# xyy7/Learning-based-RGB-D-Image-Compression

Measured on AMD Instinct MI355X. Metric: RGB-D Mpixels/s encode+decode, higher is better.
Workload: dtype f32; 1 GPU; c3_4x480x640; codec=ELIC_united ch4 q=2_2 (N=192,M=320), images_per_gpu=4, steps_per_call=4, images_per_call=16, calls=5, weights=synthetic seed 0 (stress recipe), streams=per image, y_bytes_last_batch=15943588, engine_instances=5, conv_tiles=throughput, warmup_steps_run=40, launch=HIP graph per call shape, pairs_in_flight=80

## Files before the change

### learning-based-rgb-d-image-compression_amd/csrc/common.h

```cpp
#pragma once
#include <hip/hip_runtime.h>
#include <stdint.h>
#include <stdio.h>

#define RGBD_OK 0
#define RGBD_EINVAL (-22)
#define RGBD_ENOMEM (-12)
#define RGBD_EHIP (-5)
#define RGBD_ENOSPC (-28)
#define RGBD_ESTATE (-1)

#define HIP_TRY(expr)                                                                          \
    do {                                                                                       \
        hipError_t _e = (expr);                                                                \
        if (_e != hipSuccess) {                                                                \
            fprintf(stderr, "[rgbd_amd] %s:%d %s -> %s\n", __FILE__, __LINE__, #expr,          \
                    hipGetErrorString(_e));                                                    \
            return RGBD_EHIP;                                                                  \
        }                                                                                      \
    } while (0)

struct Act {
    float* p = nullptr;
    int n = 0, h = 0, w = 0, c = 0, cs = 0;
// ... 101 lines not shown
    const long K = (long)cin_pad * taps_per_phase;
    int s;
    if (nphase == 1 && out_px_per_image <= 512) {
        if (taps_per_phase == 1) s = K >= 1500 ? 8 : (K >= 700 ? 4 : (K >= 350 ? 2 : 1));
        else s = K >= 5000 ? 8 : (K >= 1000 ? 4 : (K >= 500 ? 2 : 1));
    } else {
        s = (int)((K + 800) / 1600);
        if (s > 8) s = 8;
    }
    if (s > cin_pad / 16) s = cin_pad / 16;
    if (s < 1) s = 1;
    return s;
}

int launch_conv(const ConvArgs& a, hipStream_t s);
int conv_fused_plan(int cout_pad, int cout2_pad, int ntaps, int N, int GH, int GW, int loaded);
int launch_conv_fused(const ConvArgs& a, hipStream_t s);
int conv_log_enable(int on);
int conv_tile_override(const char* csv);
long conv_log_read(char* buf, long cap);
long conv_tile_list(int blocked, char* buf, long cap);

int launch_sigmoid_gate_ref(const float* t, int tcs, const float* mul, int mcs, const float* res2, int r2cs, float* y, int ycs,
                            int N, int HW, int C, int per_image, int threads, hipStream_t s);

int launch_nchw_to_nhwc16(const float* src, int N, int C, int H, int W, float* dst, int cs, hipStream_t s, int perm = 0);
int launch_nhwc_to_nchw_clamp(const float* src, int N, int C, int H, int W, int cs, float* dst, int clamp01,
                              hipStream_t s, int perm = 0);
int launch_maxpool7s3(const float* x, int N, int H, int W, int cs, float* y, int OH, int OW, hipStream_t s,
                      const float* x1 = nullptr, float* y1 = nullptr);
// ... 15 lines not shown
int launch_copy_channels(const float* src, int scs, float* dst, int dcs, int npix, int C, hipStream_t s);
struct SmallConvArgs {
    const float* x;
    const float* w;
    const float* bias;
    const float* res1;
    const float* mul;
    const float* res2;
    float* y;
    float* y2;
    int N, H, W, xcs, C, cin_pad, O, OH, OW, ycs, r1cs, mcs, r2cs, y2cs, K, stride, pad, act, nb;
    int ckbd;
    int kb[17];
};
int launch_small_conv_ref(const SmallConvArgs& a, hipStream_t s);
int launch_gather_taps(const float* x, int B, int h, int w, int cs, int j0, int jw, int ntap, const int* dy, const int* dx,
                       float* col, hipStream_t s);
int launch_gather_wslabs(const float* wp, int cout_pad, int ntaps_total, int cin_pad, int ntap, const int* slab, float* wout,
                         hipStream_t s);
int launch_scatter_phase(const float* src, int B, int h, int jw, int scs, int j0, int py, int px, float* dst, int OW, int dcs,
                         int C, hipStream_t s);
int launch_fill_zero(float* p, size_t n, hipStream_t s);
int launch_im2col5s2(const float* x, int N, int H, int W, int cs, int C, float* y, int OH, int OW, int KP, hipStream_t s);
int launch_layernorm(const float* x, size_t ntok, int C, int xcs, const float* w, const float* b, float* y, int ycs,
                     hipStream_t s, const float* x1 = nullptr, const float* w1 = nullptr, const float* b1 = nullptr,
                     float* y1 = nullptr);
int launch_window_attention(const float* qkv, int B, int H, int W, int C, int qcs, int heads, int shift, const float* rpb,
                            float* out, int ocs, hipStream_t s, const float* qkv1 = nullptr, const float* rpb1 = nullptr,
                            float* out1 = nullptr);
int launch_guided_window_attention(const float* q, int qcs, const float* kv, int kvcs, int B, int H, int W, int C, int heads,
                                   int shift, const float* rpb, float* out, int ocs, hipStream_t s);
int launch_patch_merge_gather(const float* x, int B, int H, int W, int C, int xcs, float* y, int ycs, hipStream_t s);
int launch_pixel_shuffle2(const float* x, int B, int H, int W, int Co, int xcs, float* y, int ycs, hipStream_t s);

struct GdnArgs {
    const float* x;
// ... 100 lines not shown
```

### learning-based-rgb-d-image-compression_amd/csrc/conv_mfma.hip

```cpp
#include <array>
#include <map>
#include <string>

#include "conv_mfma_body.h"
#include "conv_tiles.h"

bool conv_blk_tile_ok(int wm, int mt, int nt, int max_tiles);
int launch_conv_blk(const ConvArgs& a, const Choice& c, hipStream_t s);
int launch_conv_fused_blk(const ConvArgs& a, int cls, hipStream_t s);

namespace {

Choice choose(const ConvArgs& a, int max_tiles = 16)
{
    static const int cand[][3] = {{2, 3, 8}, {2, 2, 8}, {2, 5, 4}, {2, 4, 4}, {2, 3, 4}, {2, 2, 4}, {2, 1, 4}, {2, 5, 2}, {2, 4, 2},
                                  {2, 3, 2}, {2, 2, 2}, {2, 1, 2}, {2, 5, 1}, {2, 4, 1}, {2, 3, 1}, {2, 2, 1},
                                  {2, 1, 1}, {1, 3, 2}, {1, 2, 2}, {1, 1, 2}, {1, 3, 1}, {1, 2, 1}, {1, 1, 1}};
    int max_taps = 1;
    for (int p = 0; p < a.nphase; ++p) max_taps = a.taps.n[p] > max_taps ? a.taps.n[p] : max_taps;
    const double K = (double)max_taps * a.cin_pad / a.splitk;
    const int ck = a.ckbd ? 1 : 0;
    const int GWe = ck ? (a.GW + 1) / 2 : a.GW;
    Choice best{2, 4, 4, 16, 4, false};
    double best_cost = -1.0;
// ... 240 lines not shown
            p += used;
            ++n;
            if (*p == ',') ++p;
            else break;
        }
        while (*p && *p != '\n') ++p;
        if (*p == '\n') ++p;
        if (n != 14) return RGBD_EINVAL;
        char key[160];
        snprintf(key, sizeof(key), "%d,%d,%d,%d,%d,%d,%d,%d,%d", v[0], v[1], v[2], v[3], v[4], v[5], v[6], v[7], v[8]);
        g_ovr[key] = {v[9], v[10], v[11], v[12], v[13]};
    }
    return RGBD_OK;
}

int launch_conv(const ConvArgs& a_in, hipStream_t s)
{
    ConvArgs a = a_in;
    if (a.cout_store <= 0 || a.cout_store > a.cout_pad) a.cout_store = a.cout_pad;
    if (a.cout_store % 4) return RGBD_EINVAL;
    if (a.splitk < 1) a.splitk = 1;
    if (a.splitk > a.cin_pad / 16) a.splitk = a.cin_pad / 16;
    if (a.splitk > 1 && !a.partial) return RGBD_EINVAL;
    if (!conv_groups_ok(a)) return RGBD_EINVAL;
    {
        const size_t lim = (size_t)1 << 32;
        const size_t opx = (size_t)a.OH * a.OW * 4;
        const int ocs = std::max(std::max(a.ycs, a.cout_pad), std::max(a.r1cs, std::max(a.mcs, a.r2cs)));
        if ((size_t)a.H * a.W * a.xcs * 4 >= lim || opx * ocs >= lim ||
            (size_t)a.cout_pad * a.ntaps_total * a.cin_pad * 4 >= lim)
            return RGBD_EINVAL;
    }
    if (a.act == ACT_GELU && !a.partial) return RGBD_EINVAL;
    if (a.y2 && (a.partial || a.subpix || a.y2cs % 4)) return RGBD_EINVAL;
    if (a.subpix && (a.cout_pad != 16 || a.nphase != 1 || a.IS != 1 || a.OS != 2 || a.splitk > 1 || a.res1 || a.mul || a.res2 ||
                     a.ckbd || a.ycs < 4))
        return RGBD_EINVAL;
    if (a.ckbd && (a.ckbd > 2 || a.ckbd < 0 || a.nphase != 1 || a.IS != 1 || a.OS != 1)) return RGBD_EINVAL;
    const int rc = launch_conv_main(a, s);
    if (rc || !a.partial) return rc;
    const size_t total4 = (size_t)a.N * a.OH * a.OW * (a.cout_pad / 4);
    size_t g = ((a.groups == 2 ? 2 : 1) * total4 + 255) / 256;
    if (g > 2048) g = 2048;
    hipLaunchKernelGGL(splitk_reduce_kernel, dim3((unsigned)g), dim3(256), 0, s, a, total4);
    HIP_TRY(hipGetLastError());
    return RGBD_OK;
}

static int launch_conv_main(const ConvArgs& a, hipStream_t s)
{
    if (a.cin_pad % 16 || a.cout_pad % 16 || a.xcs % 4 || a.ycs % 4) return RGBD_EINVAL;
    if (a.nphase != 1 && a.nphase != 4) return RGBD_EINVAL;
    if (a.N <= 0 || a.GH <= 0 || a.GW <= 0) return RGBD_EINVAL;
    Choice c = choose(a);
    const TunedTile* t = tuned_lookup(a);
    if (t && a.blocked) {
        const int tiles = t->mt * t->nt;
        const bool ring = t->kc == 16 && (t->dma == 4 || t->dma == 5), dma = t->kc == 16 && t->dma != 0;
        if (!conv_blk_tile_ok(t->wm, t->mt, t->nt, 16) || (tiles > 12 && !ring) || (tiles > 10 && !dma)) t = nullptr;
    }
    if (t) {
// ... 103 lines not shown
```

### learning-based-rgb-d-image-compression_amd/csrc/engine.h

```cpp
#pragma once
#include <algorithm>
#include <array>
#include <cmath>
#include <cstdlib>
#include <cstring>
#include <functional>
#include <map>
#include <memory>
#include <mutex>
#include <shared_mutex>
#include <string>
#include <vector>

#include <atomic>
#include <chrono>
#include <condition_variable>
#include <dirent.h>
#include <execinfo.h>
#include <signal.h>
#include <sys/syscall.h>
#include <thread>
#include <unistd.h>

#include "../../include/rgbd_amd.h"
// ... 221 lines not shown
    int act = ACT_NONE;
    const Act* res1 = nullptr;
    const Act* mul = nullptr;
    const Act* res2 = nullptr;
    int ckbd = 0;
    const Act* dup = nullptr;
};


struct ArenaScratch {
    Arena& a;
    size_t mark() const { return a.top; }
    float* take(size_t bytes) { return (float*)a.take(bytes); }
    void release(size_t m) { a.top = m; }
};
template <class Scratch>
inline int deconv_s2_ref_run(const PackedConv& pcv, const int* rec, size_t nrec, const float* x, int B, int h, int w, int act,
                             float* out, int ocs, int tile_mode, bool launch, hipStream_t s, Scratch& scratch)
{
    const PackedConv* pc = &pcv;
    std::vector<const int*> desc(4 * (size_t)w, nullptr);
    {
        size_t pos = 0;
        for (size_t i = 0; i < desc.size(); ++i) {
            if (pos >= nrec || rec[pos] < 0 || (size_t)rec[pos] > (nrec - pos - 1) / 3) return RGBD_EINVAL;
            desc[i] = rec + pos;
            pos += 1 + 3 * (size_t)rec[pos];
        }
        if (pos != nrec) return RGBD_EINVAL;
    }
    auto same = [](const int* a, const int* b) { return a[0] == b[0] && memcmp(a, b, sizeof(int) * (1 + 3 * (size_t)a[0])) == 0; };
    for (int ph = 0; ph < 4; ++ph) {
        const int py = ph >> 1, px = ph & 1;
        for (int j0 = 0; j0 < w;) {
            const int* d = desc[(size_t)ph * w + j0];
            int j1 = j0 + 1;
            while (j1 < w && same(d, desc[(size_t)ph * w + j1])) ++j1;
            const int jw = j1 - j0, nt = d[0];
            if (nt < 1 || nt > 16) return RGBD_EINVAL;
            int dy[16], dx[16], slab[16], chain[16], nch = 0;
            for (int t = 0; t < nt; ++t) {
                const int ky = d[1 + 3 * t], kx = d[2 + 3 * t], fresh = d[3 + 3 * t];
                if (ky < 0 || ky > 4 || kx < 0 || kx > 4 || ((py + ky) & 1) || ((px + kx) & 1) || (fresh != 0 && fresh != 1)) return RGBD_EINVAL;
                dy[t] = (py + 2 - ky) / 2;
                dx[t] = (px + 2 - kx) / 2;
                slab[t] = ky * 5 + kx;
                if (fresh || t == 0) chain[nch++] = 0;
                chain[nch - 1] += pc->cin_pad;
            }
            const size_t mark = scratch.mark();
            const size_t npx = (size_t)B * h * jw;
            const int Kp = nt * pc->cin_pad;
            float* col = scratch.take(npx * Kp * sizeof(float));
            float* wsel = scratch.take((size_t)pc->cout_pad * Kp * sizeof(float));
            float* tmp = scratch.take(npx * pc->cout_pad * sizeof(float));
            float* part = nch > 1 ? scratch.take((size_t)nch * npx * pc->cout_pad * sizeof(float)) : nullptr;
            if (launch) {
                if (!col || !wsel || !tmp || (nch > 1 && !part)) return RGBD_ENOMEM;
                int r = launch_gather_taps(x, B, h, w, pc->cin_pad, j0, jw, nt, dy, dx, col, s);
                if (!r) r = launch_gather_wslabs(pc->w, pc->cout_pad, 25, pc->cin_pad, nt, slab, wsel, s);
                if (!r) {
                    PackedConv gemm;
                    gemm.w = wsel;
                    gemm.bias = pc->bias;
                    gemm.cin_pad = Kp;
                    gemm.cout_pad = pc->cout_pad;
                    gemm.k = 1;
                    ConvArgs a{};
                    conv_args_geometry(&a, gemm, col, 1, B * h, jw, Kp, tmp, pc->cout_pad, B * h, jw, 1, 0);
                    a.cout_store = pc->cout_pad;
                    a.act = act;
                    a.loaded = tile_mode;
                    a.exact_math = 1;
                    a.splitk = 1;
                    if (nch > 1) {
                        a.partial = part;
                        r = conv_set_split_ranges(&a, chain, nch);
                    }
                    if (!r) r = launch_conv(a, s);
                }
                if (!r) r = launch_scatter_phase(tmp, B, h, jw, pc->cout_pad, j0, py, px, out, 2 * w, ocs, pc->cout_pad, s);
                if (r) return r;
            }
            scratch.release(mark);
            j0 = j1;
        }
    }
    return RGBD_OK;
}

inline int small_conv_set_kblocks(SmallConvArgs* a, const int* lens, int n, int Kt)
{
    a->nb = 1;
    a->kb[0] = 0;
    a->kb[1] = Kt;
    if (!lens) return RGBD_OK;
    if (n < 1 || n > 16) return RGBD_EINVAL;
    int pos = 0;
    a->nb = n;
    for (int b = 0; b < n; ++b) {
        if (lens[b] <= 0 || lens[b] > Kt - pos) return RGBD_EINVAL;
        pos += lens[b];
        a->kb[b + 1] = pos;
// ... 20 lines not shown
        bool forward_names_z;
    };
    Modes modes() const
    {
        if (single()) return {1, {"", ""}, {"", ""}, {in_ch, in_ch}, variant == 4 ? 1 : 0, true};
        return {2, {"_r", "_d"}, {"rgb_", "depth_"}, {3, 1}, 1, false};
    }
    std::vector<int> slice_ch;
    std::map<std::string, HostTensor> raw;
    std::map<std::string, PackedConv> convs;
    std::map<std::string, float*> dense;
    TableSet tables[4];
    float* scale_table = nullptr;
    std::shared_ptr<DevGen> gen_w;
    std::shared_ptr<DevGen> gen_scale;
    bool finalized = false;

    Arena arena;
    hipStream_t s = nullptr;
    int rc = 0;
    std::map<std::string, Act> named;

    std::vector<std::vector<uint8_t>> streams[2][2];
    int32_t* dbg_sym = nullptr;
    int32_t* dbg_idx = nullptr;
    int64_t dbg_per_mod = 0;
    bool debug_floats = false;
    float* dbg_x = nullptr;
    float* dbg_s = nullptr;

// ... 1153 lines not shown
        const char* mods[2] = {"rgb", "depth"};
        const Act* in[2] = {&yr, &yd};
        Act* out[2] = {zr, zd};
        const std::string p[2] = {std::string("h_a.") + mods[0] + "_reduction.", std::string("h_a.") + mods[1] + "_reduction."};
        const Epi relu2[2] = {relu, relu}, none[2];
        const Act x0[2] = {*in[0], *in[1]};
        Act t0[2], t1[2], t2[2];
        const std::string n0[2] = {p[0] + "0", p[1] + "0"}, n2[2] = {p[0] + "2", p[1] + "2"}, n4[2] = {p[0] + "4", p[1] + "4"};
        conv2(2, n0, x0, 1, 1, relu2, nullptr, t0);
        conv2(2, n2, t0, 2, 2, relu2, nullptr, t1);
        conv2(2, n4, t1, 2, 2, none, nullptr, t2);
        *out[0] = t2[0];
        *out[1] = t2[1];
    }

    bool deconv_s2_ref(const std::string& name, const Act& x, int act, Act* out)
    {
        if (!refnum) return false;
        const PackedConv* pc = conv_of(name + ".weight");
        if (!pc || !pc->transposed || pc->k != 5 || pc->subpix || x.cs != pc->cin_pad) return false;
        const std::vector<int>* rec = ref_blocks(3, pc->cin, pc->cout, x.h, x.w);
        if (!rec) return false;
        *out = alloc(x.n, 2 * x.h, 2 * x.w, pc->cout);
        ArenaScratch scratch{arena};
        const int r = deconv_s2_ref_run(*pc, rec->data(), rec->size(), x.p, x.n, x.h, x.w, act, out->p, out->cs, tile_mode,
                                        !dry() && !rc, s, scratch);
        if (r) fail(r);
        return true;
    }

    void hs_block2(int nm, const std::string p[2], const Act own[2], const Act other[2], bool last, Act out[2])
    {
        Act f[2];
        std::string n[2];
        for (int m = 0; m < nm; ++m) {
            f[m] = alloc(own[m].n, own[m].h, own[m].w, own[m].c + other[m].c);
            se_cat_to(p[m] + ".se", own[m], other[m], f[m]);
            if (rc) return;
            n[m] = p[m] + ".deconv";
        }
        Epi e[2];
        e[0].act = e[1].act = last ? ACT_NONE : ACT_LEAKY;
        const PackedConv* pc0 = conv_of(n[0] + ".weight");
        if (nm == 2 && !last && refnum && pc0 && ref_blocks(3, pc0->cin, pc0->cout, f[0].h, f[0].w)) {
            bool ok = true;
            for (int m = 0; m < 2; ++m) ok = deconv_s2_ref(n[m], f[m], ACT_LEAKY, &out[m]) && ok;
            if (!ok) fail(RGBD_ESTATE);
            return;
        }
        conv2(nm, n, f, last ? 1 : 2, last ? 1 : 2, e, nullptr, out);
    }

    void h_s(const Act& zr, const Act& zd, Act* hr, Act* hd)
    {
        Act cur[2] = {zr, zd};
        for (int st = 1; st <= 3; ++st) {
            const std::string p[2] = {"h_s.r_h_s" + std::to_string(st), "h_s.d_h_s" + std::to_string(st)};
            const Act other[2] = {cur[1], cur[0]};
            Act o[2];
            hs_block2(2, p, cur, other, st == 3, o);
            cur[0] = o[0];
            cur[1] = o[1];
// ... 917 lines not shown
```

### learning-based-rgb-d-image-compression_amd/csrc/engine_abi.hip

```cpp
#include "engine.h"

extern "C" {

int rgbd_abi_version(void) { return RGBD_AMD_ABI_VERSION; }

static std::atomic<int> g_live_engines{0};
static std::mutex g_policy_mu;
static bool g_policy_done[64] = {false};

static int ensure_wait_policy()
{
    static const bool spin = getenv("RGBD_SPIN_WAIT") != nullptr;
    if (spin) return RGBD_OK;
    int dev = 0;
    HIP_TRY(hipGetDevice(&dev));
    std::lock_guard<std::mutex> g(g_policy_mu);
    if (dev < 0 || dev >= 64 || g_policy_done[dev]) return RGBD_OK;
    if (g_live_engines.load() == 0) {
        std::unique_lock<std::shared_mutex> cap_lk(g_capture_mu);
        HIP_TRY(hipDeviceSynchronize());
        HIP_TRY(hipSetDeviceFlags(hipDeviceScheduleBlockingSync));
    }
    g_policy_done[dev] = true;
    return RGBD_OK;
// ... 908 lines not shown
{
    if (!src || !out || !src->finalized) return RGBD_EINVAL;
    rgbd_elic* m = new rgbd_elic();
    m->N = src->N;
    m->M = src->M;
    m->slice_ch = src->slice_ch;
    m->variant = src->variant;
    m->in_ch = src->in_ch;
    m->out_ch = src->out_ch;
    m->refnum = src->refnum;
    m->ref_threads = src->ref_threads;
    m->ref_tab = src->ref_tab;
    m->convs = src->convs;
    m->dense = src->dense;
    m->gen_w = src->gen_w;
    for (int i = 0; i < 4; ++i) m->tables[i] = src->tables[i];
    m->scale_table = src->scale_table;
    m->scale_tab = src->scale_tab;
    m->gen_scale = src->gen_scale;
    m->finalized = true;
    m->is_clone = true;
    *out = m;
    ++g_live_engines;
    return RGBD_OK;
}

void rgbd_elic_destroy(rgbd_elic* m)
{
    const bool dbg = g_dbg_destroy;
    if (dbg) fprintf(stderr, "[destroy %p] wait lock\n", (void*)m);
// ... 66 lines not shown
    g->p.push_back(d);
    HIP_TRY(hipMemcpy(d, table, 64 * sizeof(float), hipMemcpyHostToDevice));
    m->scale_table = d;
    memcpy(m->scale_tab.v, table, sizeof(m->scale_tab.v));
    m->gen_scale = g;
    m->graphs_invalidate();
    return RGBD_OK;
}

static bool ends_with(const std::string& s, const char* suf)
{
    const size_t n = strlen(suf);
    return s.size() >= n && s.compare(s.size() - n, n, suf) == 0;
}

int rgbd_elic_set_ref_blocks(rgbd_elic* m, int32_t kind, int32_t cin, int32_t cout, int32_t h, int32_t w, int32_t batch,
                             const int32_t* blocks, int32_t nblocks)
{
    if (m && kind == 4 && blocks && nblocks == 1 && blocks[0] >= 1 && blocks[0] <= 4096) {
        m->ref_threads = blocks[0];
        m->graphs_invalidate();
        return RGBD_OK;
    }
    if (!m || !blocks || nblocks <= 0 || nblocks > (kind >= 2 ? 65536 : 64) || kind < 0 || kind > 3) return RGBD_EINVAL;
    int sum = 0;
    for (int i = 0; i < nblocks; ++i) {
        if (kind == 3 ? blocks[i] < 0 : (kind == 2 ? (blocks[i] < 0 || blocks[i] > 2) : blocks[i] <= 0)) return RGBD_EINVAL;
        sum += blocks[i];
    }
    if (kind == 0 && sum != cin) return RGBD_EINVAL;
    if (kind == 1 && nblocks > 16) return RGBD_EINVAL;
    if (kind == 2 && nblocks != cout) return RGBD_EINVAL;
    m->ref_tab->blocks[{kind, cin, cout, h, w, batch}] = std::vector<int>(blocks, blocks + nblocks);
    m->graphs_invalidate();
    return RGBD_OK;
}

int rgbd_elic_get_refnum(const rgbd_elic* m) { return m ? (m->refnum ? 1 : 0) : RGBD_EINVAL; }
int rgbd_elic_ref_table_misses(const rgbd_elic* m) { return m ? m->ref_tab->misses : RGBD_EINVAL; }

int rgbd_elic_finalize(rgbd_elic* m)
{
    std::unique_lock<std::shared_mutex> cap_lk(g_capture_mu);
    if (!m) return RGBD_EINVAL;
    if (m->is_clone && m->raw.empty()) return RGBD_ESTATE;
    auto gen = std::make_shared<DevGen>();
    std::map<std::string, PackedConv> convs;
    std::map<std::string, float*> dense;
    auto dev_copy = [&](const float* src, size_t n, float** out) -> int {
// ... 138 lines not shown
                const size_t no = (size_t)fi[i + 1], ni = (size_t)fi[i];
                if (mi->second.v.size() != C * no * ni || bi->second.v.size() != C * no || (i < 4 && fa->second.v.size() != C * no))
                    return RGBD_EINVAL;
                mat[i] = mi->second.v.data();
                bias[i] = bi->second.v.data();
                if (i < 4) fac[i] = fa->second.v.data();
            }
            if (ok) {
                eb_pack_cumulative(mat, bias, fac, C, prm.data());
                float* dp = nullptr;
                if (const int r = dev_copy(prm.data(), prm.size(), &dp)) return r;
                dense[pre + "cumulative"] = dp;
            }
        }
    }
    m->convs.swap(convs);
    m->dense.swap(dense);
    m->gen_w = gen;
    m->graphs_invalidate();
    m->finalized = true;
    return RGBD_OK;
}

static int check_ready(const rgbd_elic* m)
{
    if (m && m->variant == 6) return RGBD_EINVAL;
    if (!m || !m->finalized || !m->scale_table) return RGBD_ESTATE;
    for (int i = 0; i < 4; ++i)
        if (!m->tables[i].ready && !(m->single() && (i & 1))) return RGBD_ESTATE;
    return RGBD_OK;
}

int rgbd_elic_compress(rgbd_elic* m, const float* rgb_dev, const float* depth_dev, int32_t B, int32_t H, int32_t W,
// ... 246 lines not shown
```

### learning-based-rgb-d-image-compression_amd/csrc/pointwise.hip

```cpp
#include "common.h"
#include "exact_math.h"

typedef float f32x4 __attribute__((ext_vector_type(4)));

static inline unsigned grid_for(size_t work, int block = 256, unsigned cap = 256 * 8)
{
    size_t g = (work + block - 1) / block;
    if (g > cap) g = cap;
    if (g < 1) g = 1;
    return (unsigned)g;
}

__global__ void nchw_to_nhwc16_kernel(const float* __restrict__ src, int N, int C, int H, int W, float* __restrict__ dst,
                                      int cs, int perm)
{
    const size_t npix = (size_t)N * H * W;
    const int c4n = cs / 4;
    for (size_t i = blockIdx.x * (size_t)blockDim.x + threadIdx.x; i < npix * c4n; i += (size_t)gridDim.x * blockDim.x) {
        const size_t pix = i / c4n;
        const int c4 = (int)(i - pix * c4n);
        const size_t hw = pix % ((size_t)H * W);
        const size_t n = pix / ((size_t)H * W);
        f32x4 v;
#pragma unroll
// ... 517 lines not shown

int launch_se_fc_ref(const float* mean, int N, int C, int hidden, const float* w0, const float* w1, const int* cls0,
                     const int* cls1, float* hid, float* scale, hipStream_t s, int mstride, int form)
{
    const int r = launch_se_linear_ref(w0, mean, N, C, hidden, mstride > 0 ? mstride : C, 1, cls0, ACT_RELU, hid, hidden, 0, form, s);
    if (r) return r;
    return launch_se_linear_ref(w1, hid, N, hidden, C, hidden, 0, cls1, ACT_SIGMOID, scale, C, 1, form, s);
}

struct TapList {
    int n;
    int8_t dy[16], dx[16];
    uint8_t slab[16];
};

__global__ void gather_taps_kernel(const float* __restrict__ x, int B, int h, int w, int cs, int j0, int jw, TapList tl,
                                   float* __restrict__ col)
{
    const int c4n = cs / 4;
    const size_t total = (size_t)B * h * jw * tl.n * c4n;
    for (size_t i = blockIdx.x * (size_t)blockDim.x + threadIdx.x; i < total; i += (size_t)gridDim.x * blockDim.x) {
        const int c4 = (int)(i % c4n);
        size_t r = i / c4n;
        const int t = (int)(r % tl.n);
        r /= tl.n;
        const int tx = (int)(r % jw);
        r /= jw;
        const int ty = (int)(r % h);
        const size_t n = r / h;
        const int iy = ty + tl.dy[t], ix = j0 + tx + tl.dx[t];
        f32x4 v = (f32x4){0.f, 0.f, 0.f, 0.f};
        if (iy >= 0 && iy < h && ix >= 0 && ix < w) v = *reinterpret_cast<const f32x4*>(x + ((n * h + iy) * (size_t)w + ix) * cs + c4 * 4);
        *reinterpret_cast<f32x4*>(col + (((n * h + ty) * (size_t)jw + tx) * tl.n + t) * cs + c4 * 4) = v;
    }
}

__global__ void gather_wslabs_kernel(const float* __restrict__ wp, int cout_pad, int ntaps_total, int cin_pad, TapList tl,
                                     float* __restrict__ wout)
{
    const int c4n = cin_pad / 4;
    const size_t total = (size_t)cout_pad * tl.n * c4n;
    for (size_t i = blockIdx.x * (size_t)blockDim.x + threadIdx.x; i < total; i += (size_t)gridDim.x * blockDim.x) {
        const int c4 = (int)(i % c4n);
        size_t r = i / c4n;
        const int t = (int)(r % tl.n);
        const size_t co = r / tl.n;
        *reinterpret_cast<f32x4*>(wout + (co * tl.n + t) * cin_pad + c4 * 4) =
            *reinterpret_cast<const f32x4*>(wp + (co * ntaps_total + tl.slab[t]) * cin_pad + c4 * 4);
    }
}

__global__ void scatter_phase_kernel(const float* __restrict__ src, int B, int h, int jw, int scs, int j0, int py, int px,
                                     float* __restrict__ dst, int OW, int dcs, int c4n)
{
    const size_t total = (size_t)B * h * jw * c4n;
    for (size_t i = blockIdx.x * (size_t)blockDim.x + threadIdx.x; i < total; i += (size_t)gridDim.x * blockDim.x) {
        const int c4 = (int)(i % c4n);
        size_t r = i / c4n;
        const int tx = (int)(r % jw);
        r /= jw;
        const int ty = (int)(r % h);
        const size_t n = r / h;
        *reinterpret_cast<f32x4*>(dst + ((n * 2 * h + 2 * ty + py) * (size_t)OW + 2 * (j0 + tx) + px) * dcs + c4 * 4) =
            *reinterpret_cast<const f32x4*>(src + ((n * h + ty) * (size_t)jw + tx) * scs + c4 * 4);
    }
}

int launch_gather_taps(const float* x, int B, int h, int w, int cs, int j0, int jw, int ntap, const int* dy, const int* dx,
                       float* col, hipStream_t s)
{
    if (ntap < 1 || ntap > 16 || cs % 4) return RGBD_EINVAL;
    TapList tl{};
    tl.n = ntap;
    for (int t = 0; t < ntap; ++t) tl.dy[t] = (int8_t)dy[t], tl.dx[t] = (int8_t)dx[t];
    const size_t work = (size_t)B * h * jw * ntap * (cs / 4);
    hipLaunchKernelGGL(gather_taps_kernel, dim3(grid_for(work)), dim3(256), 0, s, x, B, h, w, cs, j0, jw, tl, col);
    HIP_TRY(hipGetLastError());
    return RGBD_OK;
}

int launch_gather_wslabs(const float* wp, int cout_pad, int ntaps_total, int cin_pad, int ntap, const int* slab, float* wout,
                         hipStream_t s)
{
    if (ntap < 1 || ntap > 16 || cin_pad % 4) return RGBD_EINVAL;
    TapList tl{};
    tl.n = ntap;
    for (int t = 0; t < ntap; ++t) tl.slab[t] = (uint8_t)slab[t];
    const size_t work = (size_t)cout_pad * ntap * (cin_pad / 4);
    hipLaunchKernelGGL(gather_wslabs_kernel, dim3(grid_for(work)), dim3(256), 0, s, wp, cout_pad, ntaps_total, cin_pad, tl, wout);
    HIP_TRY(hipGetLastError());
    return RGBD_OK;
}

int launch_scatter_phase(const float* src, int B, int h, int jw, int scs, int j0, int py, int px, float* dst, int OW, int dcs,
                         int C, hipStream_t s)
{
    if (C % 4 || scs % 4 || dcs % 4) return RGBD_EINVAL;
    const size_t work = (size_t)B * h * jw * (C / 4);
    hipLaunchKernelGGL(scatter_phase_kernel, dim3(grid_for(work)), dim3(256), 0, s, src, B, h, jw, scs, j0, py, px, dst, OW, dcs, C / 4);
    HIP_TRY(hipGetLastError());
    return RGBD_OK;
}


__global__ void sigmoid_gate_ref_kernel(const float* __restrict__ t, int tcs, const float* __restrict__ mul, int mcs,
                                        const float* __restrict__ res2, int r2cs, float* __restrict__ y, int ycs, int N, int HW,
                                        int C, int per_image, int threads)
{
    const int C16 = (C + 15) & ~15;
    const size_t total = (size_t)N * HW * C16;
    const long numel = (long)(per_image ? 1 : N) * C * HW;
    for (size_t i = blockIdx.x * (size_t)blockDim.x + threadIdx.x; i < total; i += (size_t)gridDim.x * blockDim.x) {
        const int sc = (int)(i % C16);
        const size_t pix = i / C16;
// ... 26 lines not shown
```

Measured before the change: 18.89 Mpx/s.

## Batch stride-2 deconv classes into grouped gather, paired GEMMs, fused finish kernel

Restructures the reference stride-2 transposed-conv path so all phase/column classes are gathered by one grouped kernel per 16 classes instead of one launch each. The two modalities run as a paired GEMM group that writes split partials. A single finish kernel sums the partials, adds bias, applies the activation and scatters into the output, replacing the per-class split-k reduce and scatter launches. Weight slabs can come from a prebuilt cache set at finalize, which removes the per-call gather_wslabs. This cuts kernel launch count and per-class scratch reuse, at the cost of more simultaneous scratch memory for all classes.

New measurement: 18.80 Mpx/s (median of 2 runs). No clear change (-0.5%).

```diff
diff --git a/learning-based-rgb-d-image-compression_amd/csrc/common.h b/learning-based-rgb-d-image-compression_amd/csrc/common.h
--- a/learning-based-rgb-d-image-compression_amd/csrc/common.h
+++ b/learning-based-rgb-d-image-compression_amd/csrc/common.h
@@ -139,6 +139,7 @@
 }
 
 int launch_conv(const ConvArgs& a, hipStream_t s);
+int launch_conv_partials(const ConvArgs& a, hipStream_t s);
 int conv_fused_plan(int cout_pad, int cout2_pad, int ntaps, int N, int GH, int GW, int loaded);
 int launch_conv_fused(const ConvArgs& a, hipStream_t s);
 int conv_log_enable(int on);
@@ -184,12 +185,24 @@
     int kb[17];
 };
 int launch_small_conv_ref(const SmallConvArgs& a, hipStream_t s);
-int launch_gather_taps(const float* x, int B, int h, int w, int cs, int j0, int jw, int ntap, const int* dy, const int* dx,
-                       float* col, hipStream_t s);
+struct DeconvClass {
+    int j0, jw, nt;
+    int py, px;
+    int planes;
+    unsigned long long col_off, part_off;
+    int8_t dy[16], dx[16];
+};
+struct DeconvClassTab {
+    static constexpr int kMax = 16;
+    int n;
+    DeconvClass c[kMax];
+};
+int launch_gather_taps_grouped(const float* x0, const float* x1, int B, int h, int w, int cs, const DeconvClassTab& tab, float* col,
+                               size_t col_set, hipStream_t s);
 int launch_gather_wslabs(const float* wp, int cout_pad, int ntaps_total, int cin_pad, int ntap, const int* slab, float* wout,
                          hipStream_t s);
-int launch_scatter_phase(const float* src, int B, int h, int jw, int scs, int j0, int py, int px, float* dst, int OW, int dcs,
-                         int C, hipStream_t s);
+int launch_deconv_finish(const float* part, size_t part_set, int B, int h, int w, int cout_pad, const DeconvClassTab& tab,
+                         const float* bias0, const float* bias1, int act, float* dst0, float* dst1, int dcs, hipStream_t s);
 int launch_fill_zero(float* p, size_t n, hipStream_t s);
 int launch_im2col5s2(const float* x, int N, int H, int W, int cs, int C, float* y, int OH, int OW, int KP, hipStream_t s);
 int launch_layernorm(const float* x, size_t ntok, int C, int xcs, const float* w, const float* b, float* y, int ycs,
diff --git a/learning-based-rgb-d-image-compression_amd/csrc/conv_mfma.hip b/learning-based-rgb-d-image-compression_amd/csrc/conv_mfma.hip
--- a/learning-based-rgb-d-image-compression_amd/csrc/conv_mfma.hip
+++ b/learning-based-rgb-d-image-compression_amd/csrc/conv_mfma.hip
@@ -278,7 +278,7 @@
     return RGBD_OK;
 }
 
-int launch_conv(const ConvArgs& a_in, hipStream_t s)
+static int launch_conv_impl(const ConvArgs& a_in, hipStream_t s, bool reduce)
 {
     ConvArgs a = a_in;
     if (a.cout_store <= 0 || a.cout_store > a.cout_pad) a.cout_store = a.cout_pad;
@@ -302,13 +302,21 @@
         return RGBD_EINVAL;
     if (a.ckbd && (a.ckbd > 2 || a.ckbd < 0 || a.nphase != 1 || a.IS != 1 || a.OS != 1)) return RGBD_EINVAL;
     const int rc = launch_conv_main(a, s);
-    if (rc || !a.partial) return rc;
+    if (rc || !a.partial || !reduce) return rc;
     const size_t total4 = (size_t)a.N * a.OH * a.OW * (a.cout_pad / 4);
     size_t g = ((a.groups == 2 ? 2 : 1) * total4 + 255) / 256;
     if (g > 2048) g = 2048;
     hipLaunchKernelGGL(splitk_reduce_kernel, dim3((unsigned)g), dim3(256), 0, s, a, total4);
     HIP_TRY(hipGetLastError());
     return RGBD_OK;
+}
+
+int launch_conv(const ConvArgs& a, hipStream_t s) { return launch_conv_impl(a, s, true); }
+
+int launch_conv_partials(const ConvArgs& a, hipStream_t s)
+{
+    if (!a.partial || a.res1 || a.mul || a.res2 || a.y2 || a.ckbd || a.bias_mode != 0) return RGBD_EINVAL;
+    return launch_conv_impl(a, s, false);
 }
 
 static int launch_conv_main(const ConvArgs& a, hipStream_t s)
diff --git a/learning-based-rgb-d-image-compression_amd/csrc/engine.h b/learning-based-rgb-d-image-compression_amd/csrc/engine.h
--- a/learning-based-rgb-d-image-compression_amd/csrc/engine.h
+++ b/learning-based-rgb-d-image-compression_amd/csrc/engine.h
@@ -259,11 +259,15 @@
     float* take(size_t bytes) { return (float*)a.take(bytes); }
     void release(size_t m) { a.top = m; }
 };
-template <class Scratch>
-inline int deconv_s2_ref_run(const PackedConv& pcv, const int* rec, size_t nrec, const float* x, int B, int h, int w, int act,
-                             float* out, int ocs, int tile_mode, bool launch, hipStream_t s, Scratch& scratch)
+
+struct DeconvProblem {
+    int j0, jw, py, px, nt, nch;
+    int dy[16], dx[16], slab[16];
+    int chain[16];
+};
+
+inline int deconv_s2_problems(const int* rec, size_t nrec, int w, int cin_pad, std::vector<DeconvProblem>* out)
 {
-    const PackedConv* pc = &pcv;
     std::vector<const int*> desc(4 * (size_t)w, nullptr);
     {
         size_t pos = 0;
@@ -275,63 +279,146 @@
         if (pos != nrec) return RGBD_EINVAL;
     }
     auto same = [](const int* a, const int* b) { return a[0] == b[0] && memcmp(a, b, sizeof(int) * (1 + 3 * (size_t)a[0])) == 0; };
+    out->clear();
     for (int ph = 0; ph < 4; ++ph) {
         const int py = ph >> 1, px = ph & 1;
         for (int j0 = 0; j0 < w;) {
             const int* d = desc[(size_t)ph * w + j0];
             int j1 = j0 + 1;
             while (j1 < w && same(d, desc[(size_t)ph * w + j1])) ++j1;
-            const int jw = j1 - j0, nt = d[0];
-            if (nt < 1 || nt > 16) return RGBD_EINVAL;
-            int dy[16], dx[16], slab[16], chain[16], nch = 0;
-            for (int t = 0; t < nt; ++t) {
+            DeconvProblem p{};
+            p.j0 = j0, p.jw = j1 - j0, p.py = py, p.px = px, p.nt = d[0];
+            if (p.nt < 1 || p.nt > 16) return RGBD_EINVAL;
+            for (int t = 0; t < p.nt; ++t) {
                 const int ky = d[1 + 3 * t], kx = d[2 + 3 * t], fresh = d[3 + 3 * t];
                 if (ky < 0 || ky > 4 || kx < 0 || kx > 4 || ((py + ky) & 1) || ((px + kx) & 1) || (fresh != 0 && fresh != 1)) return RGBD_EINVAL;
-                dy[t] = (py + 2 - ky) / 2;
-                dx[t] = (px + 2 - kx) / 2;
-                slab[t] = ky * 5 + kx;
-                if (fresh || t == 0) chain[nch++] = 0;
-                chain[nch - 1] += pc->cin_pad;
-            }
-            const size_t mark = scratch.mark();
-            const size_t npx = (size_t)B * h * jw;
-            const int Kp = nt * pc->cin_pad;
-            float* col = scratch.take(npx * Kp * sizeof(float));
-            float* wsel = scratch.take((size_t)pc->cout_pad * Kp * sizeof(float));
-            float* tmp = scratch.take(npx * pc->cout_pad * sizeof(float));
-            float* part = nch > 1 ? scratch.take((size_t)nch * npx * pc->cout_pad * sizeof(float)) : nullptr;
-            if (launch) {
-                if (!col || !wsel || !tmp || (nch > 1 && !part)) return RGBD_ENOMEM;
-                int r = launch_gather_taps(x, B, h, w, pc->cin_pad, j0, jw, nt, dy, dx, col, s);
-                if (!r) r = launch_gather_wslabs(pc->w, pc->cout_pad, 25, pc->cin_pad, nt, slab, wsel, s);
-                if (!r) {
-                    PackedConv gemm;
-                    gemm.w = wsel;
-                    gemm.bias = pc->bias;
-                    gemm.cin_pad = Kp;
-                    gemm.cout_pad = pc->cout_pad;
-                    gemm.k = 1;
-                    ConvArgs a{};
-                    conv_args_geometry(&a, gemm, col, 1, B * h, jw, Kp, tmp, pc->cout_pad, B * h, jw, 1, 0);
-                    a.cout_store = pc->cout_pad;
-                    a.act = act;
-                    a.loaded = tile_mode;
-                    a.exact_math = 1;
-                    a.splitk = 1;
-                    if (nch > 1) {
-                        a.partial = part;
-                        r = conv_set_split_ranges(&a, chain, nch);
-                    }
-                    if (!r) r = launch_conv(a, s);
+                p.dy[t] = (py + 2 - ky) / 2;
+                p.dx[t] = (px + 2 - kx) / 2;
+                p.slab[t] = ky * 5 + kx;
+                if (fresh || t == 0) p.chain[p.nch++] = 0;
+                p.chain[p.nch - 1] += cin_pad;
+            }
+            out->push_back(p);
+            j0 = j1;
+        }
+    }
+    return RGBD_OK;
+}
+
+struct DeconvSlabs {
+    typedef std::pair<const float*, std::array<uint8_t, 17>> Key;
+    std::map<Key, const float*> m;
+    static Key key(const float* w, int nt, const int* slab)
+    {
+        Key k{w, {}};
+        k.second[0] = (uint8_t)nt;
+        for (int t = 0; t < nt; ++t) k.second[1 + t] = (uint8_t)slab[t];
+        return k;
+    }
+    const float* find(const float* w, int nt, const int* slab) const
+    {
+        auto it = m.find(key(w, nt, slab));
+        return it == m.end() ? nullptr : it->second;
+    }
+};
+
+struct DeconvSet {
+    const PackedConv* pc;
+    const float* x;
+    float* out;
+};
+
+template <class Scratch>
+inline int deconv_s2_ref_run(const DeconvSet* set, int nm, const int* rec, size_t nrec, int B, int h, int w, int act, int ocs,
+                             int tile_mode, bool launch, hipStream_t s, Scratch& scratch, const DeconvSlabs* slabs = nullptr)
+{
+    if (nm < 1 || nm > 2) return RGBD_EINVAL;
+    const PackedConv* pc = set[0].pc;
+    if (nm == 2 && (set[1].pc->cin_pad != pc->cin_pad || set[1].pc->cout_pad != pc->cout_pad)) return RGBD_EINVAL;
+    std::vector<DeconvProblem> prob;
+    if (const int r = deconv_s2_problems(rec, nrec, w, pc->cin_pad, &prob)) return r;
+    std::vector<size_t> col_off(prob.size()), part_off(prob.size()), w_off(prob.size());
+    size_t col_f = 0, part_f = 0, w_f = 0;
+    for (size_t i = 0; i < prob.size(); ++i) {
+        const size_t npx = (size_t)B * h * prob[i].jw, Kp = (size_t)prob[i].nt * pc->cin_pad;
+        col_off[i] = col_f, part_off[i] = part_f, w_off[i] = w_f;
+        col_f += npx * Kp;
+        part_f += (size_t)prob[i].nch * npx * pc->cout_pad;
+        w_f += (size_t)pc->cout_pad * Kp;
+    }
+    const size_t mark = scratch.mark();
+    float* col = scratch.take(nm * col_f * sizeof(float));
+    float* part = scratch.take(nm * part_f * sizeof(float));
+    float* wsel = slabs ? nullptr : scratch.take(nm * w_f * sizeof(float));
+    if (launch) {
+        if (!col || !part || (!slabs && !wsel)) return RGBD_ENOMEM;
+        const size_t np = prob.size();
+        const DeconvSet* set1 = nm == 2 ? &set[1] : nullptr;
+        auto table = [&](size_t i0) {
+            DeconvClassTab tab{};
+            for (size_t i = i0; i < np && i < i0 + DeconvClassTab::kMax; ++i) {
+                DeconvClass& c = tab.c[tab.n++];
+                const DeconvProblem& p = prob[i];
+                c.j0 = p.j0, c.jw = p.jw, c.nt = p.nt, c.py = p.py, c.px = p.px, c.planes = p.nch;
+                c.col_off = col_off[i], c.part_off = part_off[i];
+                for (int t = 0; t < p.nt; ++t) c.dy[t] = (int8_t)p.dy[t], c.dx[t] = (int8_t)p.dx[t];
+            }
+            return tab;
+        };
+        for (size_t i0 = 0; i0 < np; i0 += DeconvClassTab::kMax)
+            if (const int r = launch_gather_taps_grouped(set[0].x, set1 ? set1->x : nullptr, B, h, w, pc->cin_pad, table(i0), col, col_f, s))
+                return r;
+        for (size_t i = 0; i < np; ++i) {
+            const DeconvProblem& p = prob[i];
+            const int Kp = p.nt * pc->cin_pad;
+            ConvArgs args[2];
+            for (int m = 0; m < nm; ++m) {
+                PackedConv gemm;
+                if (slabs) {
+                    gemm.w = const_cast<float*>(slabs->find(set[m].pc->w, p.nt, p.slab));
+                    if (!gemm.w) return RGBD_ESTATE;
+                } else {
+                    gemm.w = wsel + m * w_f + w_off[i];
+                    if (const int r = launch_gather_wslabs(set[m].pc->w, pc->cout_pad, 25, pc->cin_pad, p.nt, p.slab, gemm.w, s)) return r;
                 }
-                if (!r) r = launch_scatter_phase(tmp, B, h, jw, pc->cout_pad, j0, py, px, out, 2 * w, ocs, pc->cout_pad, s);
-                if (r) return r;
-            }
-            scratch.release(mark);
-            j0 = j1;
-        }
-    }
+                gemm.bias = set[m].pc->bias;
+                gemm.cin_pad = Kp;
+                gemm.cout_pad = pc->cout_pad;
+                gemm.k = 1;
+                ConvArgs& a = args[m];
+                a = ConvArgs{};
+                float* const planes = part + m * part_f + part_off[i];
+                conv_args_geometry(&a, gemm, col + m * col_f + col_off[i], 1, B * h, p.jw, Kp, planes, pc->cout_pad, B * h, p.jw, 1, 0);
+                a.partial = planes;
+            }
+            ConvArgs& a = args[0];
+            a.cout_store = pc->cout_pad;
+            a.loaded = tile_mode;
+            a.exact_math = 1;
+            if (nm == 2) {
+                conv_args_group1(&a, args[1]);
+                a.g1.partial = args[1].partial;
+            }
+            int r = conv_set_split_ranges(&a, p.chain, p.nch);
+            if (!r) r = launch_conv_partials(a, s);
+            if (r) return r;
+        }
+        for (size_t i0 = 0; i0 < np; i0 += DeconvClassTab::kMax)
+            if (const int r = launch_deconv_finish(part, part_f, B, h, w, pc->cout_pad, table(i0), pc->bias, set1 ? set1->pc->bias : nullptr,
+                                                   act, set[0].out, set1 ? set1->out : nullptr, ocs, s))
+                return r;
+    }
+    scratch.release(mark);
     return RGBD_OK;
+}
+
+template <class Scratch>
+inline int deconv_s2_ref_run(const PackedConv& pc, const int* rec, size_t nrec, const float* x, int B, int h, int w, int act,
+                             float* out, int ocs, int tile_mode, bool launch, hipStream_t s, Scratch& scratch,
+                             const DeconvSlabs* slabs = nullptr)
+{
+    const DeconvSet one{&pc, x, out};
+    return deconv_s2_ref_run(&one, 1, rec, nrec, B, h, w, act, ocs, tile_mode, launch, s, scratch, slabs);
 }
 
 inline int small_conv_set_kblocks(SmallConvArgs* a, const int* lens, int n, int Kt)
@@ -382,6 +469,7 @@
     float* scale_table = nullptr;
     std::shared_ptr<DevGen> gen_w;
     std::shared_ptr<DevGen> gen_scale;
+    std::shared_ptr<const DeconvSlabs> slabs;
     bool finalized = false;
 
     Arena arena;
@@ -1565,17 +1653,37 @@
         *out[1] = t2[1];
     }
 
-    bool deconv_s2_ref(const std::string& name, const Act& x, int act, Act* out)
+    bool deconv_s2_ref(const std::string& name, const Act& x, int act, Act* out) { return deconv_s2_ref(1, &name, &x, act, out); }
+    bool deconv_s2_ref(int nm, const std::string* name, const Act* x, int act, Act* out)
     {
         if (!refnum) return false;
-        const PackedConv* pc = conv_of(name + ".weight");
-        if (!pc || !pc->transposed || pc->k != 5 || pc->subpix || x.cs != pc->cin_pad) return false;
-        const std::vector<int>* rec = ref_blocks(3, pc->cin, pc->cout, x.h, x.w);
+        const PackedConv* pc[2] = {nullptr, nullptr};
+        for (int m = 0; m < nm; ++m) {
+            pc[m] = conv_of(name[m] + ".weight");
+            if (!pc[m] || !pc[m]->transposed || pc[m]->k != 5 || pc[m]->subpix || x[m].cs != pc[m]->cin_pad) return false;
+        }
+        const bool together = nm == 2 && g_pair && pc[0]->cin == pc[1]->cin && pc[0]->cout == pc[1]->cout && x[0].n == x[1].n &&
+                              x[0].h == x[1].h && x[0].w == x[1].w;
+        if (nm == 2 && !together) {
+            bool ok = true;
+            for (int m = 0; m < 2; ++m) ok = deconv_s2_ref(1, &name[m], &x[m], act, &out[m]) && ok;
+            return ok;
+        }
+        const std::vector<int>* rec = ref_blocks(3, pc[0]->cin, pc[0]->cout, x[0].h, x[0].w);
         if (!rec) return false;
-        *out = alloc(x.n, 2 * x.h, 2 * x.w, pc->cout);
+        DeconvSet set[2];
+        for (int m = 0; m < nm; ++m) {
+            out[m] = alloc(x[m].n, 2 * x[m].h, 2 * x[m].w, pc[m]->cout);
+            set[m] = DeconvSet{pc[m], x[m].p, out[m].p};
+        }
+        if (nm == 2 && out[0].cs != out[1].cs) {
+            fail(RGBD_ESTATE);
+            return true;
+        }
         ArenaScratch scratch{arena};
-        const int r = deconv_s2_ref_run(*pc, rec->data(), rec->size(), x.p, x.n, x.h, x.w, act, out->p, out->cs, tile_mode,
-                                        !dry() && !rc, s, scratch);
+        static const DeconvSlabs kNoSlabs;
+        const int r = deconv_s2_ref_run(set, nm, rec->data(), rec->size(), x[0].n, x[0].h, x[0].w, act, out[0].cs, tile_mode,
+                                        !dry() && !rc, s, scratch, slabs ? slabs.get() : &kNoSlabs);
         if (r) fail(r);
         return true;
     }
@@ -1594,9 +1702,7 @@
         e[0].act = e[1].act = last ? ACT_NONE : ACT_LEAKY;
         const PackedConv* pc0 = conv_of(n[0] + ".weight");
         if (nm == 2 && !last && refnum && pc0 && ref_blocks(3, pc0->cin, pc0->cout, f[0].h, f[0].w)) {
-            bool ok = true;
-            for (int m = 0; m < 2; ++m) ok = deconv_s2_ref(n[m], f[m], ACT_LEAKY, &out[m]) && ok;
-            if (!ok) fail(RGBD_ESTATE);
+            if (!deconv_s2_ref(2, n, f, ACT_LEAKY, out)) fail(RGBD_ESTATE);
             return;
         }
         conv2(nm, n, f, last ? 1 : 2, last ? 1 : 2, e, nullptr, out);
diff --git a/learning-based-rgb-d-image-compression_amd/csrc/engine_abi.hip b/learning-based-rgb-d-image-compression_amd/csrc/engine_abi.hip
--- a/learning-based-rgb-d-image-compression_amd/csrc/engine_abi.hip
+++ b/learning-based-rgb-d-image-compression_amd/csrc/engine_abi.hip
@@ -946,6 +946,7 @@
     m->convs = src->convs;
     m->dense = src->dense;
     m->gen_w = src->gen_w;
+    m->slabs = src->slabs;
     for (int i = 0; i < 4; ++i) m->tables[i] = src->tables[i];
     m->scale_table = src->scale_table;
     m->scale_tab = src->scale_tab;
@@ -1042,6 +1043,32 @@
     return s.size() >= n && s.compare(s.size() - n, n, suf) == 0;
 }
 
+static int build_deconv_slabs(const rgbd_elic* m, const std::map<std::string, PackedConv>& convs, DevGen* gen, DeconvSlabs* have)
+{
+    bool launched = false;
+    for (const auto& kv : convs) {
+        const PackedConv& pc = kv.second;
+        if (!pc.transposed || pc.k != 5 || pc.subpix) continue;
+        for (const auto& rt : m->ref_tab->blocks) {
+            if (rt.first[0] != 3 || rt.first[1] != pc.cin || rt.first[2] != pc.cout || rt.first[4] <= 0) continue;
+            std::vector<DeconvProblem> prob;
+            if (deconv_s2_problems(rt.second.data(), rt.second.size(), rt.first[4], pc.cin_pad, &prob)) continue;
+            for (const DeconvProblem& p : prob) {
+                const DeconvSlabs::Key key = DeconvSlabs::key(pc.w, p.nt, p.slab);
+                if (have->m.count(key)) continue;
+                float* d = nullptr;
+                HIP_TRY(hipMalloc((void**)&d, (size_t)pc.cout_pad * p.nt * pc.cin_pad * sizeof(float)));
+                gen->p.push_back(d);
+                if (const int r = launch_gather_wslabs(pc.w, pc.cout_pad, 25, pc.cin_pad, p.nt, p.slab, d, nullptr)) return r;
+                launched = true;
+                have->m[key] = d;
+            }
+        }
+    }
+    if (launched) HIP_TRY(hipStreamSynchronize(nullptr));
+    return RGBD_OK;
+}
+
 int rgbd_elic_set_ref_blocks(rgbd_elic* m, int32_t kind, int32_t cin, int32_t cout, int32_t h, int32_t w, int32_t batch,
                              const int32_t* blocks, int32_t nblocks)
 {
@@ -1061,6 +1088,13 @@
     if (kind == 2 && nblocks != cout) return RGBD_EINVAL;
     m->ref_tab->blocks[{kind, cin, cout, h, w, batch}] = std::vector<int>(blocks, blocks + nblocks);
     m->graphs_invalidate();
+    if (kind == 3 && m->finalized && m->refnum && m->gen_w) {
+        std::unique_lock<std::shared_mutex> cap_lk(g_capture_mu);
+        auto slabs = std::make_shared<DeconvSlabs>();
+        if (m->slabs) *slabs = *m->slabs;
+        if (const int r = build_deconv_slabs(m, m->convs, m->gen_w.get(), slabs.get())) return r;
+        m->slabs = slabs;
+    }
     return RGBD_OK;
 }
 
@@ -1229,9 +1263,13 @@
             }
         }
     }
+    auto slabs = std::make_shared<DeconvSlabs>();
+    if (m->refnum)
+        if (const int r = build_deconv_slabs(m, convs, gen.get(), slabs.get())) return r;
     m->convs.swap(convs);
     m->dense.swap(dense);
     m->gen_w = gen;
+    m->slabs = slabs;
     m->graphs_invalidate();
     m->finalized = true;
     return RGBD_OK;
diff --git a/learning-based-rgb-d-image-compression_amd/csrc/pointwise.hip b/learning-based-rgb-d-image-compression_amd/csrc/pointwise.hip
--- a/learning-based-rgb-d-image-compression_amd/csrc/pointwise.hip
+++ b/learning-based-rgb-d-image-compression_amd/csrc/pointwise.hip
@@ -555,27 +555,6 @@
     uint8_t slab[16];
 };
 
-__global__ void gather_taps_kernel(const float* __restrict__ x, int B, int h, int w, int cs, int j0, int jw, TapList tl,
-                                   float* __restrict__ col)
-{
-    const int c4n = cs / 4;
-    const size_t total = (size_t)B * h * jw * tl.n * c4n;
-    for (size_t i = blockIdx.x * (size_t)blockDim.x + threadIdx.x; i < total; i += (size_t)gridDim.x * blockDim.x) {
-        const int c4 = (int)(i % c4n);
-        size_t r = i / c4n;
-        const int t = (int)(r % tl.n);
-        r /= tl.n;
-        const int tx = (int)(r % jw);
-        r /= jw;
-        const int ty = (int)(r % h);
-        const size_t n = r / h;
-        const int iy = ty + tl.dy[t], ix = j0 + tx + tl.dx[t];
-        f32x4 v = (f32x4){0.f, 0.f, 0.f, 0.f};
-        if (iy >= 0 && iy < h && ix >= 0 && ix < w) v = *reinterpret_cast<const f32x4*>(x + ((n * h + iy) * (size_t)w + ix) * cs + c4 * 4);
-        *reinterpret_cast<f32x4*>(col + (((n * h + ty) * (size_t)jw + tx) * tl.n + t) * cs + c4 * 4) = v;
-    }
-}
-
 __global__ void gather_wslabs_kernel(const float* __restrict__ wp, int cout_pad, int ntaps_total, int cin_pad, TapList tl,
                                      float* __restrict__ wout)
 {
@@ -591,31 +570,96 @@
     }
 }
 
-__global__ void scatter_phase_kernel(const float* __restrict__ src, int B, int h, int jw, int scs, int j0, int py, int px,
-                                     float* __restrict__ dst, int OW, int dcs, int c4n)
-{
-    const size_t total = (size_t)B * h * jw * c4n;
+__global__ void gather_taps_grouped_kernel(const float* __restrict__ x0, const float* __restrict__ x1, int B, int h, int w, int cs,
+                                           DeconvClassTab tab, float* __restrict__ colbase, size_t col_set)
+{
+    const DeconvClass& c = tab.c[blockIdx.y];
+    const int c4n = cs / 4, jw = c.jw, nt = c.nt;
+    const float* __restrict__ x = blockIdx.z ? x1 : x0;
+    float* __restrict__ col = colbase + blockIdx.z * col_set + c.col_off;
+    const size_t total = (size_t)B * h * jw * nt * c4n;
     for (size_t i = blockIdx.x * (size_t)blockDim.x + threadIdx.x; i < total; i += (size_t)gridDim.x * blockDim.x) {
         const int c4 = (int)(i % c4n);
         size_t r = i / c4n;
+        const int t = (int)(r % nt);
+        r /= nt;
         const int tx = (int)(r % jw);
         r /= jw;
         const int ty = (int)(r % h);
         const size_t n = r / h;
-        *reinterpret_cast<f32x4*>(dst + ((n * 2 * h + 2 * ty + py) * (size_t)OW + 2 * (j0 + tx) + px) * dcs + c4 * 4) =
-            *reinterpret_cast<const f32x4*>(src + ((n * h + ty) * (size_t)jw + tx) * scs + c4 * 4);
-    }
-}
-
-int launch_gather_taps(const float* x, int B, int h, int w, int cs, int j0, int jw, int ntap, const int* dy, const int* dx,
-                       float* col, hipStream_t s)
-{
-    if (ntap < 1 || ntap > 16 || cs % 4) return RGBD_EINVAL;
-    TapList tl{};
-    tl.n = ntap;
-    for (int t = 0; t < ntap; ++t) tl.dy[t] = (int8_t)dy[t], tl.dx[t] = (int8_t)dx[t];
-    const size_t work = (size_t)B * h * jw * ntap * (cs / 4);
-    hipLaunchKernelGGL(gather_taps_kernel, dim3(grid_for(work)), dim3(256), 0, s, x, B, h, w, cs, j0, jw, tl, col);
+        const int iy = ty + c.dy[t], ix = c.j0 + tx + c.dx[t];
+        f32x4 v = (f32x4){0.f, 0.f, 0.f, 0.f};
+        if (iy >= 0 && iy < h && ix >= 0 && ix < w) v = *reinterpret_cast<const f32x4*>(x + ((n * h + iy) * (size_t)w + ix) * cs + c4 * 4);
+        *reinterpret_cast<f32x4*>(col + (((n * h + ty) * (size_t)jw + tx) * nt + t) * cs + c4 * 4) = v;
+    }
+}
+
+__global__ void deconv_finish_kernel(const float* __restrict__ partbase, size_t part_set, int B, int h, int w, int cp,
+                                     DeconvClassTab tab, const float* __restrict__ bias0, const float* __restrict__ bias1, int act,
+                                     float* __restrict__ dst0, float* __restrict__ dst1, int dcs)
+{
+    const DeconvClass& c = tab.c[blockIdx.y];
+    const int c4n = cp / 4, jw = c.jw;
+    const float* __restrict__ part = partbase + blockIdx.z * part_set + c.part_off;
+    const float* __restrict__ bias = blockIdx.z ? bias1 : bias0;
+    float* __restrict__ dst = blockIdx.z ? dst1 : dst0;
+    const size_t npx = (size_t)B * h * jw, total = npx * c4n, plane = npx * cp;
+    for (size_t i = blockIdx.x * (size_t)blockDim.x + threadIdx.x; i < total; i += (size_t)gridDim.x * blockDim.x) {
+        const size_t pix = i / c4n;
+        const int cb = (int)(i - pix * c4n) * 4;
+        f32x4 v = *reinterpret_cast<const f32x4*>(part + pix * cp + cb);
+        for (int s = 1; s < c.planes; ++s) v += *reinterpret_cast<const f32x4*>(part + s * plane + pix * cp + cb);
+        v += *reinterpret_cast<const f32x4*>(bias + cb);
+        if (act == ACT_RELU) {
+#pragma unroll
+            for (int e = 0; e < 4; ++e) v[e] = fmaxf(v[e], 0.f);
+        } else if (act == ACT_LEAKY) {
+#pragma unroll
+            for (int e = 0; e < 4; ++e) v[e] = v[e] > 0.f ? v[e] : v[e] * 0.01f;
+        }
+        size_t r = pix;
+        const int tx = (int)(r % jw);
+        r /= jw;
+        const int ty = (int)(r % h);
+        const size_t n = r / h;
+        *reinterpret_cast<f32x4*>(dst + ((n * 2 * h + 2 * ty + c.py) * (size_t)(2 * w) + 2 * (c.j0 + tx) + c.px) * dcs + cb) = v;
+    }
+}
+
+static int deconv_tab_ok(const DeconvClassTab& tab, int h, int w)
+{
+    if (tab.n < 1 || tab.n > DeconvClassTab::kMax) return RGBD_EINVAL;
+    for (int i = 0; i < tab.n; ++i) {
+        const DeconvClass& c = tab.c[i];
+        if (c.nt < 1 || c.nt > 16 || c.jw < 1 || c.j0 < 0 || c.j0 + c.jw > w || c.planes < 1 || c.planes > 16 || (c.py & ~1) || (c.px & ~1))
+            return RGBD_EINVAL;
+    }
+    return h > 0 ? RGBD_OK : RGBD_EINVAL;
+}
+
+int launch_gather_taps_grouped(const float* x0, const float* x1, int B, int h, int w, int cs, const DeconvClassTab& tab, float* col,
+                               size_t col_set, hipStream_t s)
+{
+    if (cs % 4 || B <= 0 || !x0 || !col || col_set % 4 || deconv_tab_ok(tab, h, w)) return RGBD_EINVAL;
+    size_t work = 0;
+    for (int i = 0; i < tab.n; ++i) work = std::max(work, (size_t)B * h * tab.c[i].jw * tab.c[i].nt * (cs / 4));
+    hipLaunchKernelGGL(gather_taps_grouped_kernel, dim3(grid_for(work), tab.n, x1 ? 2 : 1), dim3(256), 0, s, x0, x1, B, h, w, cs, tab,
+                       col, col_set);
+    HIP_TRY(hipGetLastError());
+    return RGBD_OK;
+}
+
+int launch_deconv_finish(const float* part, size_t part_set, int B, int h, int w, int cout_pad, const DeconvClassTab& tab,
+                         const float* bias0, const float* bias1, int act, float* dst0, float* dst1, int dcs, hipStream_t s)
+{
+    if (cout_pad % 4 || dcs % 4 || dcs < cout_pad || B <= 0 || !part || !bias0 || !dst0 || !bias1 != !dst1 || part_set % 4 ||
+        deconv_tab_ok(tab, h, w))
+        return RGBD_EINVAL;
+    if (act != ACT_NONE && act != ACT_RELU && act != ACT_LEAKY) return RGBD_EINVAL;
+    size_t work = 0;
+    for (int i = 0; i < tab.n; ++i) work = std::max(work, (size_t)B * h * tab.c[i].jw * (cout_pad / 4));
+    hipLaunchKernelGGL(deconv_finish_kernel, dim3(grid_for(work), tab.n, dst1 ? 2 : 1), dim3(256), 0, s, part, part_set, B, h, w,
+                       cout_pad, tab, bias0, bias1, act, dst0, dst1, dcs);
     HIP_TRY(hipGetLastError());
     return RGBD_OK;
 }
@@ -629,16 +673,6 @@
     for (int t = 0; t < ntap; ++t) tl.slab[t] = (uint8_t)slab[t];
     const size_t work = (size_t)cout_pad * ntap * (cin_pad / 4);
     hipLaunchKernelGGL(gather_wslabs_kernel, dim3(grid_for(work)), dim3(256), 0, s, wp, cout_pad, ntaps_total, cin_pad, tl, wout);
-    HIP_TRY(hipGetLastError());
-    return RGBD_OK;
-}
-
-int launch_scatter_phase(const float* src, int B, int h, int jw, int scs, int j0, int py, int px, float* dst, int OW, int dcs,
-                         int C, hipStream_t s)
-{
-    if (C % 4 || scs % 4 || dcs % 4) return RGBD_EINVAL;
-    const size_t work = (size_t)B * h * jw * (C / 4);
-    hipLaunchKernelGGL(scatter_phase_kernel, dim3(grid_for(work)), dim3(256), 0, s, src, B, h, jw, scs, j0, py, px, dst, OW, dcs, C / 4);
     HIP_TRY(hipGetLastError());
     return RGBD_OK;
 }
```
